# chlhnu/DOT-SOCP

Hardware: AMD Instinct MI355X
Metric: ADMM iters/sec on NxNxT dot2d staggered grid at 1/2/4/8 MI355X (higher is better)
Workload: dtype f64

## Files before the change

dot-socp_amd/capi.py:

```python
import ctypes
import os

import numpy as np

_HERE = os.path.dirname(os.path.abspath(__file__))
LIB_PATH = os.path.join(_HERE, "lib", "libdotsocp.so")

i64 = ctypes.c_longlong
dbl = ctypes.c_double
vp = ctypes.c_void_p


class DotsocpError(RuntimeError):
    def __init__(self, code, msg):
        super().__init__(f"libdotsocp error {code}: {msg}")
        self.code = code


class Problem(ctypes.Structure):
    _fields_ = [("dim", ctypes.c_int), ("weighted", ctypes.c_int),
                ("ny", i64), ("nx", i64), ("nt", i64),
                ("D", dbl), ("E", dbl), ("cScale", dbl), ("dScale", dbl),
                ("normc", dbl), ("normd", dbl)]

# ... 82 lines not shown
    "dotsocp_bfd_conj_dev": (ctypes.c_int, [vp, vp, i64, i64, i64, dbl, vp]),
    "dotsocp_create": (vp, [ctypes.POINTER(Problem), ctypes.c_int, ctypes.c_int]),
    "dotsocp_create_multi": (vp, [ctypes.POINTER(Problem), ctypes.c_int, ctypes.c_int]),
    "dotsocp_destroy": (None, [vp]),
    "dotsocp_rccl_unique_id": (ctypes.c_int, [vp]),
    "dotsocp_attach_rccl": (ctypes.c_int, [vp, vp, ctypes.c_int, ctypes.c_int]),
    "dotsocp_slab_range": (ctypes.c_int, [i64, ctypes.c_int, ctypes.c_int, ctypes.POINTER(i64), ctypes.POINTER(i64)]),
    "dotsocp_field_len": (i64, [ctypes.POINTER(Problem), ctypes.c_int]),
    "dotsocp_dct_algorithm": (ctypes.c_int, [i64]),
    "dotsocp_dct_levels": (ctypes.c_int, [i64, ctypes.c_int]),
    "dotsocp_cdft_levels": (ctypes.c_int, [i64]),
    "dotsocp_tsolve_tri_safe": (ctypes.c_int, [i64, i64, i64]),
    "dotsocp_cone_writes_beta": (ctypes.c_int, [i64, dbl, i64, ctypes.c_int, ctypes.c_int, ctypes.c_int, dbl, dbl]),
    "dotsocp_rescale_due": (ctypes.c_int, [i64, ctypes.c_int, dbl, dbl]),
    "dotsocp_qcone_form": (ctypes.c_int, [i64, dbl, i64, ctypes.c_int, ctypes.c_int, ctypes.c_int, ctypes.c_int, dbl, dbl]),
    "dotsocp_release_cache": (i64, []),
    "dotsocp_upload": (ctypes.c_int, [vp, ctypes.c_int, vp]),
    "dotsocp_upload_layers": (ctypes.c_int, [vp, ctypes.c_int, vp, i64, i64]),
    "dotsocp_download": (ctypes.c_int, [vp, ctypes.c_int, vp]),
    "dotsocp_begin": (ctypes.c_int, [vp, ctypes.POINTER(Opts)]),
    "dotsocp_begin_method": (ctypes.c_int, [vp, ctypes.POINTER(Opts), ctypes.c_int, ctypes.POINTER(AccOpts)]),
    "dotsocp_run": (ctypes.c_int, [vp, i64, ctypes.POINTER(i64)]),
    "dotsocp_recover_outputs": (ctypes.c_int, [vp, vp, vp, vp, vp, vp, vp, vp, vp]),
    "dotsocp_report_edges": (ctypes.c_int, [vp]),
    "dotsocp_solution_report": (ctypes.c_int, [vp, vp, vp, ctypes.POINTER(Report), vp, vp]),
    "dotsocp_recover_velocity": (ctypes.c_int, [vp, vp, vp, dbl, vp, vp]),
    "dotsocp_advect_particles": (ctypes.c_int, [vp, vp, vp, ctypes.POINTER(AdvectOpts), vp, vp, vp, vp, ctypes.POINTER(i64)]),
    "dotsocp_push_mass": (ctypes.c_int, [vp, vp, vp, ctypes.POINTER(PushOpts), vp, vp, vp, vp, vp, ctypes.POINTER(i64),
                                         ctypes.POINTER(dbl), vp]),
    "dotsocp_map_report": (ctypes.c_int, [vp, vp, vp, ctypes.POINTER(AdvectOpts), vp, vp, vp, ctypes.POINTER(MapReport),
# ... 107 lines not shown
```

dot-socp_amd/csrc/capi.hip:

```cpp
#include <cstring>
#include <new>

#include "comm.h"
#include "image_table.h"
#include "solver.h"
#include "weights.h"

using namespace dotsocp;

namespace dotsocp {
extern thread_local std::string g_last_error;
int dotsocp_slab_range_impl(i64 nt, int world, int rank, i64 *t0, i64 *t1);
}

struct dotsocp_ctx {
    Solver s;
};

struct dotsocp_weights {
    Weights w;
};

static int require_device() {
    int n = 0;
// ... 263 lines not shown
int dotsocp_cdft_levels(dotsocp_i64 n) { return cdft_levels(n); }
int dotsocp_tsolve_tri_safe(dotsocp_i64 ny, dotsocp_i64 nx, dotsocp_i64 nt) { return tsolve_tri_safe(ny, nx, nt) ? 1 : 0; }

int dotsocp_cone_writes_beta(dotsocp_i64 it, double last_sigma_it, dotsocp_i64 maxit, int check_step_by_step,
                             int last_of_run, int rescale, double maxFeas, double relGap) {
    return cone_writes_beta(it, last_sigma_it, maxit, check_step_by_step != 0, last_of_run != 0, rescale, maxFeas, relGap) ? 1 : 0;
}
int dotsocp_rescale_due(dotsocp_i64 it, int rescale, double maxFeas, double relGap) {
    return rescale_due(it, rescale, maxFeas, relGap) ? 1 : 0;
}
int dotsocp_qcone_form(dotsocp_i64 it, double last_sigma_it, dotsocp_i64 maxit, int check_step_by_step, int last_of_run,
                       int next_last_of_run, int rescale, double maxFeas, double relGap) {
    return qcone_form(it, last_sigma_it, maxit, check_step_by_step != 0, last_of_run != 0, next_last_of_run != 0, rescale,
                      maxFeas, relGap);
}

dotsocp_i64 dotsocp_field_len(const dotsocp_problem *p, int field) {
    if (!p || (p->dim != 1 && p->dim != 2) || p->nt < 2 || p->nx < 1 || (p->dim == 2 && p->ny < 1)) return -1;
    const i64 ny = p->dim == 1 ? p->nx : p->ny, nx = p->dim == 1 ? 1 : p->nx, nt = p->nt;
    const i64 Nphi = ny * nx * nt, Nz = ny * nx * (nt - 1);
    const i64 Nq = Nz + ny * (nx - 1) * nt + (ny - 1) * nx * nt;
    switch (field) {
        case DOTSOCP_F_PHI: case DOTSOCP_F_C: return Nphi;
        case DOTSOCP_F_Q: case DOTSOCP_F_ALPHA: case DOTSOCP_F_WEIGHT: return Nq;
        case DOTSOCP_F_Z: case DOTSOCP_F_BETA: return Nz * (p->dim == 1 ? 6 : 10);
        default: return -1;
    }
}

int dotsocp_upload(dotsocp_ctx *ctx, int field, const double *host) { CTX_OR_FAIL(); return ctx->s.upload(field, host); }
// ... 223 lines not shown
```

dot-socp_amd/csrc/fused.hip:

```cpp
#include "device_utils.h"
#include "gather_tile.h"
#include "kernels.h"

#include <cstdlib>

namespace dotsocp {

template <int MODE, int XB, bool NT = false, bool GIN = false, bool GOUT = false>
__global__ void __launch_bounds__(64 * XB) k_cone_fused(Grid g, LoopCoef c, FusedArgs a) {
    static_assert(MODE == 1 || !(GIN || GOUT), "the gamma form exists between two MODE_B passes only");
    constexpr bool DUAL = (MODE >= 5);
    constexpr bool UPD = (MODE != 0 && MODE != 6);
    constexpr bool PROJ = (MODE < 2 || MODE >= 5);
    __shared__ double2 xch[2][XB][64];
    __shared__ double2 xchp[DUAL ? 2 : 1][DUAL ? XB : 1][DUAL ? 64 : 1];
    const int lane = threadIdx.x, xl = threadIdx.y;
    const BlockId blk = block_id(a.xcd != 0);
    const i64 y = (i64)blk.x * 64 + lane;
    const i64 x = (i64)blk.y * XB + xl;
    const bool inb = (y < g.ny) && (x < g.nx);
    const i64 yc = inb ? y : 0, xc = inb ? x : 0;
    const i64 t0 = ((i64)blk.z + a.z0) * a.TC;
    const i64 t1 = (t0 + a.TC < g.ncl) ? t0 + a.TC : g.ncl;
    const bool lastChunk = (t1 == g.ncl);
    constexpr bool GATHER = (PROJ || MODE == 4);
    const bool carried = GATHER && !DUAL && t0 > 0 && a.carry_in != nullptr;
    const i64 tstart = (GATHER && t0 > 0 && !carried) ? t0 - 1 : t0;
    const i64 nxblk = gridDim.y, nyblk = gridDim.x;

    EdgeQuad cur = load_edges(g, a.q, yc, xc, tstart, c.sf), curo, cur3;
    if (UPD && !GIN) curo = load_edges(g, a.q_old, yc, xc, tstart, c.sf);
    if (MODE == 5) cur3 = load_edges(g, a.q3, yc, xc, tstart, c.sf);
    GatherCarry gc, gcp;
    if (carried) {
        const i64 ci = yc + g.py * xc;
        gc.p3 = a.carry_in[ci]; gc.p4 = a.carry_in[g.plane + ci];
        gc.p7 = a.carry_in[2 * g.plane + ci]; gc.p8 = a.carry_in[3 * g.plane + ci];
    }
// ... 111 lines not shown
    fg.nxblk = (g.nx + fg.XB - 1) / fg.XB;
    const i64 tiles = fg.nyblk * fg.nxblk;
    const i64 target = 2048;
    i64 chunks = (target + tiles - 1) / tiles;
    if (chunks < 1) chunks = 1;
    if (!(g.first && g.last) && cone_split_enabled() && chunks < 2 && g.ncl >= 12) chunks = 2;
    i64 TC = (g.ncl + chunks - 1) / chunks;
    if (TC < 8) TC = 8;
    if (TC > g.ncl) TC = g.ncl;
    if (TC < 1) TC = 1;
    fg.TC = TC;
    fg.chunks = (g.ncl + TC - 1) / TC;
    fg.sx_len = (g.ncl + 1) * fg.nxblk * g.ny;
    fg.sy_len = (g.ncl + 1) * g.nx * fg.nyblk;
    return 0;
}

int launch_cone_fused(int mode, const Grid &g, const LoopCoef &c, const FusedGeom &fg, FusedArgs a,
                      hipStream_t st, i64 z0, i64 zcount, int flavour) {
    if (g.Nz <= 0) return 0;
    if (zcount < 0) zcount = fg.chunks - z0;
    if (z0 < 0 || zcount <= 0 || z0 + zcount > fg.chunks) return 0;
    a.TC = fg.TC;
    a.z0 = (int)z0;
    a.xcd = tile_xcd_remap(g) ? 1 : 0;
    dim3 grid((unsigned)fg.nyblk, (unsigned)fg.nxblk, (unsigned)zcount);
    dim3 blk(64, 4);
    const bool nt = stream_nt_enabled();
#define CONE_MODE(M)                                                                     \
    case M:                                                                              \
// ... 27 lines not shown
```

dot-socp_amd/csrc/kernels.h:

```cpp
#pragma once
#include "common.h"
#include "defer.h"
#include "particle_block.h"

namespace dotsocp {

struct LoopCoef {
    double s;
    double sf;
    double dF;
    double at, ax, ay;
    double tau;
    double c1, c2;
    double dinv1, dinv2;
};

enum {
    S_Q2 = 0, S_Z2, S_APHI2, S_ALPHA2, S_BETA2, S_FBBETA2, S_PRIM1, S_PRIM2, S_DUAL1, S_DUAL2,
    S_COMPLEM, S_DOTCOMP, S_RHO2, S_RHOFQ2, S_MRHOB, S_M2, S_RHOB2, S_QALPHA, S_CPHI, S_PHI2,
    S_COUNT
};

struct KktCoef {
    double sigma;
// ... 37 lines not shown
    const double *q_old;
    const double *q;
    const double *beta_in;
    double *beta_out;
    double *z_out;
    double *q2;
    double *sx, *sy;
    const double *q3;
    double *p2, *sxp, *syp;
    i64 TC;
    ScaleOps bops;
    int xcd;
    int z0;
    const double *carry_in;
    double *carry_out;
};
bool tile_xcd_remap(const Grid &g);
int fused_geometry(const Grid &g, FusedGeom &fg);
enum { CONE_GIN = 1, CONE_GOUT = 2 };
int launch_cone_fused(int mode, const Grid &g, const LoopCoef &c, const FusedGeom &fg, FusedArgs a,
                      hipStream_t st, i64 z0 = 0, i64 zcount = -1, int flavour = 0);
bool cone_split_enabled();

struct KktWork;
struct AccArgs {
    const double *q;
    const double *z_in, *beta_in;
    const double *z0, *beta0;
    double *z0_out, *beta0_out;
    double bdiv;
    KktCoef kk;
// ... 103 lines not shown
    int c_ends;
};
int launch_qstep_rhs(const Grid &g, const LoopCoef &c, const FusedGeom &fg, const double *phi, const double *q2,
                     const double *sx, const double *sy, const double *weight, const double *tail_bx,
                     const double *tail_by, const double *cvec, double *q_out, const double *alpha_in, double *alpha_out,
                     double *rhs, hipStream_t st, i64 z0 = 0, i64 zcount = -1, i64 zstride = 1,
                     const QStepExtra *ex = nullptr);
i64 qstep_rhs_blocks(const Grid &g, const FusedGeom &fg);
struct QConeArgs {
    const double *phi, *q2v, *sx, *sy, *cvec, *alpha_in, *gamma_in;
    double *alpha_out, *rhs, *q_out, *beta_out, *q2_out, *sx_out, *sy_out;
    i64 TC;
    int ap_on;
    double ap_mul, ap_div;
    int c_ends;
};
int launch_qcone(const Grid &g, const LoopCoef &c, const FusedGeom &fg, QConeArgs a, bool gout, hipStream_t st);
i64 qcone_chunk_len(const Grid &g);
i64 qstep_rhs_chunks(const Grid &g, const FusedGeom &fg, i64 *TC = nullptr);
int launch_qstep_rhs_acc(int var, const Grid &g, const LoopCoef &c, const FusedGeom &fg, const double *phi,
                         const double *q2, const double *sx, const double *sy, const double *weight, const double *cvec,
                         double *q_raw, const double *alpha_in, double *alpha_out, double *rhs, double *q_state,
                         const double *q_anchor, const double *alpha_anchor, const AccCoef &k, hipStream_t st,
                         const double *tail_bx = nullptr, const double *tail_by = nullptr, double *u0_tail = nullptr);
int launch_qstep_palm_first(const Grid &g, const LoopCoef &c, const FusedGeom &fg, const double *phi, const double *q2,
                            const double *sx, const double *sy, const double *cvec, double *q_out, const double *alpha,
                            double *rhs, hipStream_t st, const double *tail_bx = nullptr, const double *tail_by = nullptr,
                            const double *qk = nullptr);

int launch_qstep_fused(const Grid &g, const LoopCoef &c, const FusedGeom &fg, const double *phi,
                       const double *q2, const double *sx, const double *sy, const double *weight,
                       const double *tail_bx, const double *tail_by, double *q_out, double *alpha,
// ... 98 lines not shown
```

dot-socp_amd/csrc/qstep_march.hip:

```cpp
#include "device_utils.h"
#include "gather_tile.h"
#include "kernels.h"
#include "qstep_tile.h"

#include <cstdlib>

namespace dotsocp {


struct QRhsArgs {
    const double *phi, *q2v, *sx, *sy, *weight, *tail_bx, *tail_by, *cvec, *alpha_in;
    double *q_out, *alpha_out, *rhs;
    double *u0_tail;
    i64 TC, z0, zstride;
    double *q_state;
    const double *q_anchor, *alpha_anchor;
    double c1, c2, om_rho, rho;
    APend ap;
    int xcd;
    const double *qk;
    double *partials, *resid;
    double kappa, dsD;
    int c_ends;
};
// ... 252 lines not shown
#define QRHS_LAUNCH(W, V) DS_KLAUNCH((k_qstep_rhs<W, V>), grid, blk, 0, st, g, c, fg, a)
    if (var == 0 && a.partials) {
        if (a.weight) DS_KLAUNCH((k_qstep_rhs<true, 0, true>), grid, blk, 0, st, g, c, fg, a);
        else DS_KLAUNCH((k_qstep_rhs<false, 0, true>), grid, blk, 0, st, g, c, fg, a);
    } else if (a.weight) {
        if (var == 0) QRHS_LAUNCH(true, 0); else if (var == 1) QRHS_LAUNCH(true, 1); else QRHS_LAUNCH(true, 2);
    } else {
        if (var == 0) QRHS_LAUNCH(false, 0); else if (var == 1) QRHS_LAUNCH(false, 1);
        else if (var == 2) QRHS_LAUNCH(false, 2); else QRHS_LAUNCH(false, 3);
    }
#undef QRHS_LAUNCH
    DS_HIP(hipGetLastError());
    return 0;
}

template <bool NT, bool GOUT>
__global__ void __launch_bounds__(TILE_Y *TILE_X, 3) k_qcone(Grid g, LoopCoef c, FusedGeom fg, QConeArgs a) {
    constexpr int XB = TILE_X;
    __shared__ double2 xch[2][XB][TILE_Y];
    __shared__ double ph[2][XB + 2][TILE_Y + 2];
    __shared__ double2 gch[2][XB][64];
    const APend ap{a.ap_on, a.ap_mul, a.ap_div};
    const BlockId blk = block_id(true);
    const QTile<XB> t = q_tile<XB>(g, fg, blk);
    const int lane = t.lane, xl = t.xl;
    const i64 y = t.y, x = t.x;
    const bool inb = t.inb;
    const i64 t0 = (i64)blk.z * a.TC;
    const i64 t1 = (t0 + a.TC < g.ntl) ? t0 + a.TC : g.ntl;
    const i64 tstart = (t0 >= 2) ? t0 - 2 : 0;
    const i64 tstop = (t1 == g.ntl) ? t1 + 1 : t1;
    const i64 nxblk = gridDim.y, nyblk = gridDim.x;
    const QSrc src{a.phi, a.q2v, a.sx, a.sy, nullptr, nullptr, nullptr, a.cvec, a.alpha_in, nullptr, a.c_ends};
    double p0 = 0.0;
    if (inb) {
        const i64 node0 = y + g.py * (x + g.nx * tstart);
        p0 = a.phi[node0];
        store_phi_layer<XB>(ph[0], t, p0, load_phi_halo(g, t, a.phi, node0));
    }
    double u0prev = 0.0;
    double q0c = 0.0;
    EdgeQuad eprev{0.0, 0.0, 0.0, 0.0};
    GatherCarry gc;
    int par = 0;
    __syncthreads();
    for (i64 tl = tstart; tl < tstop; ++tl) {
        const bool own = tl >= t0;
        const bool hasC = (tl > tstart) && (tl - 1 < g.ncl);
        const i64 ci = t.yc + g.py * (t.xc + g.nx * (hasC ? tl - 1 : 0));
        double b[10];
        if (hasC) {
#pragma unroll
            for (int j = 0; j < 10; ++j) b[j] = ld_stream<NT>(a.gamma_in + j * g.Nc + ci);
        }
        EdgeQuad ecur{0.0, 0.0, 0.0, 0.0};
        double q0n = 0.0;
        if (tl < g.ntl) {
            const QLayerIn in = q_layer_load<false, XB>(g, c, fg, t, src, ph[par], tl, false, false);
            const QLayerOut o = q_layer_calc<false, 0, XB>(c, t, in, ap, p0, false, false);
            q0n = o.q0n;
            if (own) {
                if (in.hasCell) {
                    a.alpha_out[in.node] = o.a0n;
                    if (!GOUT) a.q_out[in.node] = o.q0n;
                }
                if (t.hasBx) {
                    a.alpha_out[in.eX] = o.aXn;
                    if (!GOUT) a.q_out[in.eX] = o.qXn;
                }
                if (t.hasBy) {
                    a.alpha_out[in.eY] = o.aYn;
                    if (!GOUT) a.q_out[in.eY] = o.qYn;
                }
            }
            xch[par][xl][lane] = make_double2(o.ubx, o.qXn);
            store_phi_layer<XB>(ph[par ^ 1], t, in.pTl, in.h);
            __syncthreads();
            const double uby_s = __shfl_up(o.uby, 1, 64);
            const double qY_s = __shfl_up(o.qYn, 1, 64);
            if (inb) {
                const double2 r = from_left(t, xch[par], make_double2(o.ubx_l, o.qL),
                                            make_double2(0.0, 0.0));
                const double uby_m = from_below(t, uby_s, o.uby_b), qY_m = from_below(t, qY_s, o.qB);
                if (own) a.rhs[in.node] = adjoint_sum(g, c, t, tl, u0prev, o.u0, r.x, o.ubx, uby_m, o.uby) + in.cv;
                ecur.xm = (x >= 1) ? c.sf * r.y : 0.0;
                ecur.xp = (x <= g.nx - 2) ? c.sf * o.qXn : 0.0;
                ecur.ym = (y >= 1) ? c.sf * qY_m : 0.0;
                ecur.yp = (y <= g.ny - 2) ? c.sf * o.qYn : 0.0;
            }
            u0prev = o.u0;
            p0 = o.pT;
            par ^= 1;
        }
        if (tl > tstart) {
            double w[10];
            if (hasC) {
                double v[10];
                build_z2(v, q0c, eprev, ecur, c.s, c.dF);
#pragma unroll
                for (int j = 0; j < 10; ++j) b[j] = mult_finish(b[j], v[j], c.tau);
                if (!GOUT && own && inb) {
#pragma unroll
                    for (int j = 0; j < 10; ++j) st_stream<NT>(a.beta_out + j * g.Nc + ci, b[j]);
                }
#pragma unroll
                for (int j = 0; j < 10; ++j) v[j] = v[j] - b[j];
                proj_row<10>(v);
                if (GOUT && own && inb) {
// ... 1 lines not shown
                    for (int j = 0; j < 10; ++j) st_stream<NT>(a.beta_out + j * g.Nc + ci, mult_carry(b[j], v[j], c.tau));
                }
#pragma unroll
                for (int j = 0; j < 10; ++j) w[j] = v[j] + b[j];
                if (own && inb) a.q2_out[ci] = c.s * (w[9] - w[0]);
            } else {
#pragma unroll
                for (int j = 0; j < 10; ++j) w[j] = 0.0;
            }
            gather_emit<XB>(g, c.sf, gch, gc, w, tl - 1, own && inb, x, y, xl, lane, nxblk, nyblk, blk.y, blk.x, a.q2_out,
                            a.sx_out, a.sy_out);
        }
        eprev = ecur;
        q0c = q0n;
    }
}

i64 qcone_chunk_len(const Grid &g) {
    i64 TC = g.ntl;
    if (const char *e = getenv("DOTSOCP_QCONE_TC")) {
        const i64 n = atoll(e);
        if (n >= 1) TC = n;
    }
    return TC < g.ntl ? TC : g.ntl;
}

int launch_qcone(const Grid &g, const LoopCoef &c, const FusedGeom &fg, QConeArgs a, bool gout, hipStream_t st) {
    if (fg.XB != TILE_X || !(g.first && g.last) || g.ncl < 1) { set_error("internal: k_qcone on a grid it does not serve"); return DOTSOCP_ESTATE; }
    a.TC = qcone_chunk_len(g);
    const i64 chunks = (g.ntl + a.TC - 1) / a.TC;
    dim3 grid((unsigned)fg.nyblk, (unsigned)fg.nxblk, (unsigned)chunks);
    dim3 blk(TILE_Y, TILE_X);
    const bool nt = stream_nt_enabled();
    if (gout) {
        if (nt) DS_KLAUNCH((k_qcone<true, true>), grid, blk, 0, st, g, c, fg, a);
        else DS_KLAUNCH((k_qcone<false, true>), grid, blk, 0, st, g, c, fg, a);
    } else {
        if (nt) DS_KLAUNCH((k_qcone<true, false>), grid, blk, 0, st, g, c, fg, a);
        else DS_KLAUNCH((k_qcone<false, false>), grid, blk, 0, st, g, c, fg, a);
    }
    DS_HIP(hipGetLastError());
    return 0;
}

int launch_qstep_palm_first(const Grid &g, const LoopCoef &c, const FusedGeom &fg, const double *phi, const double *q2,
                            const double *sx, const double *sy, const double *cvec, double *q_out, const double *alpha,
                            double *rhs, hipStream_t st, const double *tail_bx, const double *tail_by, const double *qk) {
    QRhsArgs a{};
// ... 7 lines not shown
```

dot-socp_amd/csrc/solver.h:

```cpp
#pragma once
#include <chrono>
#include <functional>
#include <memory>
#include <string>
#include <type_traits>
#include <vector>

#include "hostmem.h"
#include "kernels.h"

namespace dotsocp {

constexpr unsigned long long POISON_WORD = 0x7ff8bad0bad0bad0ull;
int guarded_malloc(void **p, size_t bytes, bool fp = false);
void guarded_free(void *p);
bool poison_enabled();
int poison_region(void *p, size_t bytes);
long long device_cache_release();
long long device_cache_held(int dev);
int canary_check(std::string *report);
bool canary_enabled();
bool stream_stress_enabled();
void stream_stress(hipStream_t st);

// ... 221 lines not shown
    bool deferred = false;
    bool z_valid = true;
    bool z_prev_ok = false;
    bool rhs_valid = false;
    bool cone_carry = true;
    bool beta_gamma = false;
    bool cone_gout = false;
    bool last_of_run = false;
    int qcone = -1;
    bool q_valid = true;
    bool early_pass = false;
    bool early_gout = false;
    bool next_last_of_run = false;
    int need_q(const char *who) const;
    int qcone_decide() const;
    bool time_limit_passed() const;
    i64 timeout_at = -1;
    bool timeout_pending = false;
    int need_beta_form(const char *who) const;
    ScaleOps bops{0, 1.0, 1.0, 1.0, 1.0};
    ScaleOps zp_ops{0, 1.0, 1.0, 1.0, 1.0};
    int push_beta_op(double mul, double div);
    int flush_beta();
    ScaleOps aops{0, 1.0, 1.0, 1.0, 1.0};
    int flush_alpha();
    int sigma_scale_folded(double factor);
    FusedArgs pending_step_args(const Slab &s) const;
    double last_S[S_COUNT] = {0};
    double last_S_sigma = 1.0;
    i64 last_S_it = -1;
// ... 73 lines not shown
```

dot-socp_amd/csrc/solver.hip:

```cpp
#include "solver.h"

#include <algorithm>
#include <cmath>
#include <cstring>

#include "comm.h"

namespace dotsocp {

void Solver::update_coef() {
    lc.s = E / D;
    lc.sf = edge_factor(lc.s);
    lc.dF = E / dScale;
    const double ht = 1.0 / (double)(nt - 1);
    lc.at = D * (1.0 / ht);
    lc.ax = (nx > 1) ? D * (1.0 / (1.0 / (double)(nx - 1))) : 0.0;
    lc.ay = (ny > 1) ? D * (1.0 / (1.0 / (double)(ny - 1))) : 0.0;
    lc.tau = opts.tau;
    const double tmp = (E / D) * (E / D);
    if (prob.weighted) { lc.c1 = 2.0 * tmp; lc.c2 = tmp; }
    else { lc.c1 = 1.0 + 2.0 * tmp; lc.c2 = 1.0 + tmp; }
    lc.dinv1 = 1.0 / lc.c1;
    lc.dinv2 = 1.0 / lc.c2;
}
// ... 246 lines not shown
        DS_CHECK(flush_alpha());
        FOR_SLABS(s) DS_CHECK(launch_rhs(s.g, lc, s.q, s.alpha, s.c, s.weight, s.u0_prev, s.w0, s.st, c_ends_on && s.c_ends));
    } else if (multi()) {
        FOR_SLABS(s)
            if (!s.g.first) DS_CHECK(launch_rhs_fixup(s.g, lc, s.u0_prev, s.w0, s.st));
    }
    rhs_valid = false;
    prof_end(PH_RHS);
    prof_begin(PH_POISSON);
    DS_CHECK(poisson_all(hooks));
    prof_end(PH_POISSON);
    return 0;
}

int Solver::phase_z(int part) {
    if (early_pass) {
        early_pass = false;
        if (part != 0 || !fused || !deferred || cone_gout != early_gout) {
            set_error("internal: the early cone pass wrote %s, the schedule asks for %s", early_gout ? "gamma" : "beta",
                      cone_gout ? "gamma" : "beta");
            return DOTSOCP_ESTATE;
        }
        return 0;
    }
    DS_CHECK(need_q("phase_z"));
    if (part != 1) DS_CHECK(ensure_halo());
    if (!fused) {
        prof_begin(PH_PROJ);
        FOR_SLABS(s) DS_CHECK(launch_cone_proj(s.g, lc, s.q, s.beta, s.z, s.st));
        prof_end(PH_PROJ);
        return 0;
    }
    const bool gin = beta_gamma, gout = deferred && cone_gout;
    if (gin && (!deferred || !bops.empty())) {
        set_error("internal: gamma form %s", deferred ? "with a pending scaling of beta" : "without a pending multiplier step");
        return DOTSOCP_ESTATE;
    }
    const int flavour = (gin ? CONE_GIN : 0) | (gout ? CONE_GOUT : 0);
    const int ph = deferred ? (gin ? PH_CONE_CARRY : PH_FUSED_B) : PH_FUSED_A;
    z_valid = false;
// ... 3 lines not shown
        FusedArgs a{};
        a.q = s.q;
        a.q2 = s.q2;
        a.sx = s.sx;
        a.sy = s.sy;
        a.beta_in = s.beta;
        a.bops = bops;
        const i64 C = s.fg.chunks;
        const i64 z0 = (part == 2) ? C - 1 : 0;
        const i64 zc = (part == 0) ? C : ((part == 1) ? C - 1 : 1);
        if (deferred) {
            a.q_old = s.q_old;
            a.beta_out = s.beta2;
        }
        const int mode = deferred ? 1 : 0;
        if (s.carry && C > 1) {
            for (i64 z = z0; z < z0 + zc; ++z) {
                a.carry_in = (z > 0) ? s.carry : nullptr;
                a.carry_out = (z + 1 < C) ? s.carry : nullptr;
                DS_CHECK(launch_cone_fused(mode, s.g, lc, s.fg, a, s.st, z, 1, flavour));
            }
        } else {
            DS_CHECK(launch_cone_fused(mode, s.g, lc, s.fg, a, s.st, z0, zc, flavour));
        }
        if (deferred && part != 1) std::swap(s.beta, s.beta2);
    }
    prof_end(ph);
    if (part == 1) return 0;
    if (deferred) {
        bops.clear();
        beta_gamma = gout;
    }
    return 0;
}

KktCoef Solver::kkt_coef() const {
    KktCoef k;
    k.sigma = sigma;
    k.kappa = sigma * cScale * D;
    k.dsD = dScale / D;
    k.dsE = dScale / E;
    return k;
}

int Solver::phase_q(int part, bool kkt, int early) {
    if (!fused) DS_CHECK(flush_alpha());
    if (early != QCONE_NONE && (part != 0 || kkt || multi() || !fused || !deferred || !beta_gamma || !bops.empty())) {
        set_error("internal: early cone pass in a state it does not serve");
        return DOTSOCP_ESTATE;
    }
    const bool egout = (early == QCONE_STEADY);
    const int ph = (early != QCONE_NONE) ? PH_QCONE : PH_QSTEP;
    prof_begin(ph);
    FOR_SLABS(s) {
        hipStream_t st = s.st;
        if (early != QCONE_NONE && qcone != 2) {
            if (!s.sx2) {
                DS_CHECK(s.zalloc(&s.sx2, s.fg.sx_len));
                DS_CHECK(s.zalloc(&s.sy2, s.fg.sy_len));
            }
            QConeArgs a{};
            a.phi = s.phi; a.q2v = s.q2; a.sx = s.sx; a.sy = s.sy; a.cvec = s.c; a.alpha_in = s.alpha; a.gamma_in = s.beta;
            a.alpha_out = s.alpha2; a.rhs = s.w0; a.q_out = s.q_old; a.beta_out = s.beta2;
            a.q2_out = s.q; a.sx_out = s.sx2; a.sy_out = s.sy2;
            a.ap_on = aops.n; a.ap_mul = aops.mul; a.ap_div = aops.div;
            a.c_ends = (c_ends_on && s.c_ends) ? 1 : 0;
            DS_CHECK(launch_qcone(s.g, lc, s.fg, a, egout, st));
            std::swap(s.alpha, s.alpha2);
            std::swap(s.q, s.q_old);
            std::swap(s.q2, s.q_old);
            std::swap(s.sx, s.sx2);
// ... 8 lines not shown
            else if (part == 2) { z0 = C - 1; zc = 1; }
            QStepExtra ex{};
            ex.aops = aops;
            ex.c_ends = (c_ends_on && s.c_ends) ? 1 : 0;
            if (multi() && !s.g.last && part != 1) ex.u0_tail = s.send_plane;
            if (kkt) {
                const KktCoef k = kkt_coef();
                ex.partials = kkt_qstep_partials(s.g, s.kw);
                ex.resid = s.w1;
                ex.kappa = k.kappa; ex.dsD = k.dsD;
            }
            DS_CHECK(launch_qstep_rhs(s.g, lc, s.fg, s.phi, s.q2, s.sx, s.sy, s.weight, s.tail_bx, s.tail_by, s.c,
                                      s.q_old, s.alpha, s.alpha2, s.w0, st, z0, zc, zs, &ex));
            if (part != 1) std::swap(s.alpha, s.alpha2);
            if (part != 1) std::swap(s.q, s.q_old);
            if (early != QCONE_NONE) {
                FusedArgs a{};
                a.q = s.q; a.q2 = s.q2; a.sx = s.sx; a.sy = s.sy;
                a.beta_in = s.beta; a.beta_out = s.beta2;
                a.bops = bops;
                DS_CHECK(launch_cone_fused(1, s.g, lc, s.fg, a, s.st, 0, s.fg.chunks, CONE_GIN | (egout ? CONE_GOUT : 0)));
                std::swap(s.beta, s.beta2);
            }
        }
    }
    prof_end(ph);
    if (part == 1) return 0;
    q_valid = true;
    if (early != QCONE_NONE) {
        q_valid = !egout || qcone == 2;
        beta_gamma = egout;
        z_valid = false;
        z_prev_ok = false;
        early_pass = true;
        early_gout = egout;
    }
    u0_made = multi() && fused;
    if (fused) aops.clear();
    rhs_valid = fused;
    if (multi() && fused && comm_z && cone_split_enabled()) halo_pending = true;
    else DS_CHECK(exchange_q_halo(true));
    return 0;
}

int Solver::phase_mult() {
    if (fused) {
// ... 216 lines not shown
    if (last_of_run) return true;
    return rescale_due(it + 1, rescale, maxFeas, relGap);
}

int qcone_form(i64 it, double lastSigmaIt, i64 maxit, bool checkStepByStep, bool last_of_run, bool next_last_of_run,
               int rescale, double maxFeas, double relGap) {
    if (cone_writes_beta(it, lastSigmaIt, maxit, checkStepByStep, last_of_run, rescale, maxFeas, relGap)) return QCONE_NONE;
    return cone_writes_beta(it + 1, lastSigmaIt, maxit, checkStepByStep, next_last_of_run, rescale, maxFeas, relGap)
               ? QCONE_EXIT : QCONE_STEADY;
}

bool Solver::time_limit_passed() const {
    return timeout_pending || (remote() ? false : (elapsed() > time_limit || (timeout_at > 0 && it >= timeout_at)));
}

int Solver::qcone_decide() const {
    if (qcone == 0 || !fused || multi() || prob.weighted || method != DOTSOCP_METHOD_INPALM) return QCONE_NONE;
    if (!deferred || !beta_gamma || !bops.empty()) return QCONE_NONE;
    const Slab &s = slabs[0];
    if (s.g.ncl < 1 || s.fg.XB != 4) return QCONE_NONE;
    if (qcone < 0 && s.fg.nyblk * s.fg.nxblk < 2048) return QCONE_NONE;
    if (time_limit_passed()) return QCONE_NONE;
    return qcone_form(it, lastSigmaIt, opts.maxit, opts.ifCheckStepByStep != 0, last_of_run, next_last_of_run, rescale,
                      maxFeas, relGap);
}

bool if_adjust_sigma(double iter, double last_iter) {
    const double passed = iter - last_iter;
    if (iter < 20 && passed >= 3) return true;
    if (iter < 50 && passed >= 6) return true;
    if (iter < 100 && passed >= 10) return true;
    if (iter < 200 && passed >= 15) return true;
    if (iter < 500 && passed >= 25) return true;
    return passed >= 40;
}
// ... 130 lines not shown
            if (split) DS_CHECK(phase_z(2));
            return make_tails();
        };
        hooks.behind = [&]() -> int { return async_comm([&]() { return send_tails(); }, EV_JOIN); };
        DS_CHECK(phase_phi(&hooks));
    } else {
        DS_CHECK(phase_phi());
        DS_CHECK(phase_z(0));
    }
    if (fold) {
        FOR_SLABS(s) DS_CHECK(clear_partials(s));
    }
    if (inter) {
        DS_CHECK(async_comm([&]() { return send_phi_head(); }, EV_HALO));
        DS_CHECK(comm_wait(EV_JOIN));
        if (split_q) DS_CHECK(phase_q(1, fold));
        DS_CHECK(comm_wait(EV_HALO));
        DS_CHECK(phase_q(split_q ? 2 : 0, fold));
    } else {
        DS_CHECK(ship_tails());
        DS_CHECK(phase_q(0, fold, fold ? QCONE_NONE : qcone_decide()));
    }
    DS_CHECK(phase_mult());
    const bool timed_out = time_limit_passed();
    timeout_pending = false;
    if (timed_out && (beta_gamma || early_pass)) {
        timeout_pending = true;
        return 0;
    }
    if (kkt_due || timed_out)
        DS_CHECK(kkt_block(adjustSigmaYes, timed_out, brk, fold));
    return 0;
}
// ... 132 lines not shown
```

include/dotsocp.h:

```cpp
#ifndef DOTSOCP_H
#define DOTSOCP_H

#ifdef __cplusplus
extern "C" {
#endif

typedef long long dotsocp_i64;

enum {
    DOTSOCP_OK = 0,
    DOTSOCP_EINVAL = -1,
    DOTSOCP_ENODEVICE = -2,
    DOTSOCP_EHIP = -3,
    DOTSOCP_ESTATE = -4,
    DOTSOCP_ECOMM = -5
};

const char *dotsocp_last_error(void);
const char *dotsocp_version(void);
int dotsocp_device_count(void);
dotsocp_i64 dotsocp_release_cache(void);


int dotsocp_proj_soc(double *out, const double *in, dotsocp_i64 M, dotsocp_i64 K);
// ... 87 lines not shown
dotsocp_i64 dotsocp_field_len(const dotsocp_problem *prob, int field);

int dotsocp_dct_algorithm(dotsocp_i64 n);

int dotsocp_cdft_levels(dotsocp_i64 n);

int dotsocp_dct_levels(dotsocp_i64 n, int axis);

int dotsocp_tsolve_tri_safe(dotsocp_i64 ny, dotsocp_i64 nx, dotsocp_i64 nt);

int dotsocp_cone_writes_beta(dotsocp_i64 it, double last_sigma_it, dotsocp_i64 maxit, int check_step_by_step,
                             int last_of_run, int rescale, double maxFeas, double relGap);
int dotsocp_rescale_due(dotsocp_i64 it, int rescale, double maxFeas, double relGap);
int dotsocp_qcone_form(dotsocp_i64 it, double last_sigma_it, dotsocp_i64 maxit, int check_step_by_step, int last_of_run,
                       int next_last_of_run, int rescale, double maxFeas, double relGap);

int dotsocp_upload(dotsocp_ctx *ctx, int field, const double *host);
int dotsocp_download(dotsocp_ctx *ctx, int field, double *host);
int dotsocp_upload_layers(dotsocp_ctx *ctx, int field, const double *host, dotsocp_i64 t0, dotsocp_i64 n);

int dotsocp_begin(dotsocp_ctx *ctx, const dotsocp_opts *opts);
int dotsocp_begin_method(dotsocp_ctx *ctx, const dotsocp_opts *opts, int method, const dotsocp_acc_opts *acc);
int dotsocp_run(dotsocp_ctx *ctx, dotsocp_i64 n_iters, dotsocp_i64 *done);
int dotsocp_finish(dotsocp_ctx *ctx, dotsocp_result *res);

int dotsocp_recover_outputs(dotsocp_ctx *ctx, const double *rho0, const double *rho1, double *rho, double *Ex,
                            double *Ey, double *q0, double *bx, double *by);

#define DOTSOCP_REPORT_BINS 49
#define DOTSOCP_REPORT_RHO_FLOOR 1e-8
// ... 136 lines not shown
```

Measured before the change: 98.98.

## Extend fused q-step/cone early pass to multi-GPU slabs with split launches

Enables the fused qcone early pass, which combines the q-step and the cone projection, when the grid is split into slabs across multiple GPUs. The interior slab part runs the fused kernel before the halo arrives. The remaining tail layers are projected by a partial cone launch with t_begin/t_end bounds and a carry buffer. The aim is to remove a separate full cone pass and its memory traffic on multi-device runs, at the cost of more launch bookkeeping and schedule state.

```diff
diff --git a/dot-socp_amd/capi.py b/dot-socp_amd/capi.py
--- a/dot-socp_amd/capi.py
+++ b/dot-socp_amd/capi.py
@@ -120,6 +120,7 @@
     "dotsocp_cone_writes_beta": (ctypes.c_int, [i64, dbl, i64, ctypes.c_int, ctypes.c_int, ctypes.c_int, dbl, dbl]),
     "dotsocp_rescale_due": (ctypes.c_int, [i64, ctypes.c_int, dbl, dbl]),
     "dotsocp_qcone_form": (ctypes.c_int, [i64, dbl, i64, ctypes.c_int, ctypes.c_int, ctypes.c_int, ctypes.c_int, dbl, dbl]),
+    "dotsocp_cone_rest_launch": (ctypes.c_int, [i64, i64, i64, i64, ctypes.POINTER(i64), ctypes.POINTER(ctypes.c_int)]),
     "dotsocp_release_cache": (i64, []),
     "dotsocp_upload": (ctypes.c_int, [vp, ctypes.c_int, vp]),
     "dotsocp_upload_layers": (ctypes.c_int, [vp, ctypes.c_int, vp, i64, i64]),
diff --git a/dot-socp_amd/csrc/capi.hip b/dot-socp_amd/csrc/capi.hip
--- a/dot-socp_amd/csrc/capi.hip
+++ b/dot-socp_amd/csrc/capi.hip
@@ -301,6 +301,15 @@
     return qcone_form(it, last_sigma_it, maxit, check_step_by_step != 0, last_of_run != 0, next_last_of_run != 0, rescale,
                       maxFeas, relGap);
 }
+int dotsocp_cone_rest_launch(dotsocp_i64 ncl, dotsocp_i64 tc, dotsocp_i64 first, dotsocp_i64 z, dotsocp_i64 *t_begin,
+                             int *carried) {
+    i64 tb = 0;
+    int cr = 0;
+    const bool on = cone_rest_launch(ncl, tc, first, z, &tb, &cr);
+    if (t_begin) *t_begin = on ? tb : -1;
+    if (carried) *carried = on ? cr : 0;
+    return on ? 1 : 0;
+}
 
 dotsocp_i64 dotsocp_field_len(const dotsocp_problem *p, int field) {
     if (!p || (p->dim != 1 && p->dim != 2) || p->nt < 2 || p->nx < 1 || (p->dim == 2 && p->ny < 1)) return -1;
diff --git a/dot-socp_amd/csrc/fused.hip b/dot-socp_amd/csrc/fused.hip
--- a/dot-socp_amd/csrc/fused.hip
+++ b/dot-socp_amd/csrc/fused.hip
@@ -20,8 +20,10 @@
     const i64 x = (i64)blk.y * XB + xl;
     const bool inb = (y < g.ny) && (x < g.nx);
     const i64 yc = inb ? y : 0, xc = inb ? x : 0;
-    const i64 t0 = ((i64)blk.z + a.z0) * a.TC;
-    const i64 t1 = (t0 + a.TC < g.ncl) ? t0 + a.TC : g.ncl;
+    const i64 tc0 = ((i64)blk.z + a.z0) * a.TC;
+    const i64 t0 = (a.t_begin > tc0) ? a.t_begin : tc0;
+    const i64 tce = (a.t_end > 0 && a.t_end < g.ncl) ? a.t_end : g.ncl;
+    const i64 t1 = (tc0 + a.TC < tce) ? tc0 + a.TC : tce;
     const bool lastChunk = (t1 == g.ncl);
     constexpr bool GATHER = (PROJ || MODE == 4);
     const bool carried = GATHER && !DUAL && t0 > 0 && a.carry_in != nullptr;
@@ -163,6 +165,16 @@
     fg.sx_len = (g.ncl + 1) * fg.nxblk * g.ny;
     fg.sy_len = (g.ncl + 1) * g.nx * fg.nyblk;
     return 0;
+}
+
+bool cone_rest_launch(i64 ncl, i64 TC, i64 first, i64 z, i64 *t_begin, int *carried) {
+    if (TC < 1 || z < 0 || first < 0 || first >= ncl) return false;
+    const i64 c0 = z * TC, c1 = (c0 + TC < ncl) ? c0 + TC : ncl;
+    if (c0 >= ncl || c1 <= first) return false;
+    const i64 tb = (first > c0) ? first : c0;
+    if (t_begin) *t_begin = tb;
+    if (carried) *carried = (tb > 0) ? 1 : 0;
+    return true;
 }
 
 int launch_cone_fused(int mode, const Grid &g, const LoopCoef &c, const FusedGeom &fg, FusedArgs a,
diff --git a/dot-socp_amd/csrc/kernels.h b/dot-socp_amd/csrc/kernels.h
--- a/dot-socp_amd/csrc/kernels.h
+++ b/dot-socp_amd/csrc/kernels.h
@@ -75,7 +75,9 @@
     int z0;
     const double *carry_in;
     double *carry_out;
-};
+    i64 t_begin, t_end;
+};
+bool cone_rest_launch(i64 ncl, i64 TC, i64 first, i64 z, i64 *t_begin, int *carried);
 bool tile_xcd_remap(const Grid &g);
 int fused_geometry(const Grid &g, FusedGeom &fg);
 enum { CONE_GIN = 1, CONE_GOUT = 2 };
@@ -209,8 +211,12 @@
     int ap_on;
     double ap_mul, ap_div;
     int c_ends;
-};
-int launch_qcone(const Grid &g, const LoopCoef &c, const FusedGeom &fg, QConeArgs a, bool gout, hipStream_t st);
+    const double *tail_bx, *tail_by;
+    double *carry_out;
+    i64 t_lo, t_hi;
+};
+int launch_qcone(const Grid &g, const LoopCoef &c, const FusedGeom &fg, QConeArgs a, bool gout, hipStream_t st, i64 z0 = 0,
+                 i64 zcount = -1);
 i64 qcone_chunk_len(const Grid &g);
 i64 qstep_rhs_chunks(const Grid &g, const FusedGeom &fg, i64 *TC = nullptr);
 int launch_qstep_rhs_acc(int var, const Grid &g, const LoopCoef &c, const FusedGeom &fg, const double *phi,
diff --git a/dot-socp_amd/csrc/qstep_march.hip b/dot-socp_amd/csrc/qstep_march.hip
--- a/dot-socp_amd/csrc/qstep_march.hip
+++ b/dot-socp_amd/csrc/qstep_march.hip
@@ -290,7 +290,7 @@
     return 0;
 }
 
-template <bool NT, bool GOUT>
+template <bool NT, bool GOUT, bool SLAB = false>
 __global__ void __launch_bounds__(TILE_Y *TILE_X, 3) k_qcone(Grid g, LoopCoef c, FusedGeom fg, QConeArgs a) {
     constexpr int XB = TILE_X;
     __shared__ double2 xch[2][XB][TILE_Y];
@@ -302,12 +302,14 @@
     const int lane = t.lane, xl = t.xl;
     const i64 y = t.y, x = t.x;
     const bool inb = t.inb;
-    const i64 t0 = (i64)blk.z * a.TC;
-    const i64 t1 = (t0 + a.TC < g.ntl) ? t0 + a.TC : g.ntl;
+    const i64 thi = SLAB ? a.t_hi : g.ntl;
+    const i64 t0 = (SLAB ? a.t_lo : 0) + (i64)blk.z * a.TC;
+    const i64 t1 = (t0 + a.TC < thi) ? t0 + a.TC : thi;
     const i64 tstart = (t0 >= 2) ? t0 - 2 : 0;
     const i64 tstop = (t1 == g.ntl) ? t1 + 1 : t1;
     const i64 nxblk = gridDim.y, nyblk = gridDim.x;
-    const QSrc src{a.phi, a.q2v, a.sx, a.sy, nullptr, nullptr, nullptr, a.cvec, a.alpha_in, nullptr, a.c_ends};
+    const QSrc src{a.phi, a.q2v, a.sx, a.sy, nullptr, SLAB ? a.tail_bx : nullptr, SLAB ? a.tail_by : nullptr, a.cvec, a.alpha_in,
+                   nullptr, a.c_ends};
     double p0 = 0.0;
     if (inb) {
         const i64 node0 = y + g.py * (x + g.nx * tstart);
@@ -320,7 +322,50 @@
     GatherCarry gc;
     int par = 0;
     __syncthreads();
-    for (i64 tl = tstart; tl < tstop; ++tl) {
+    auto qpart = [&](const i64 tl, const bool own, const bool tails, EdgeQuad &ecur, double &q0n) {
+        const QLayerIn in = q_layer_load<false, XB>(g, c, fg, t, src, ph[par], tl, tails, false);
+        const QLayerOut o = q_layer_calc<false, 0, XB>(c, t, in, ap, p0, tails, false);
+        q0n = o.q0n;
+        const bool qst = !GOUT || (SLAB && (tl == 0 || tl == thi - 1));
+        if (own) {
+            if (in.hasCell) {
+                a.alpha_out[in.node] = o.a0n;
+                if (qst) a.q_out[in.node] = o.q0n;
+            }
+            if (t.hasBx) {
+                a.alpha_out[in.eX] = o.aXn;
+                if (qst) a.q_out[in.eX] = o.qXn;
+            }
+            if (t.hasBy) {
+                a.alpha_out[in.eY] = o.aYn;
+                if (qst) a.q_out[in.eY] = o.qYn;
+            }
+        }
+        xch[par][xl][lane] = make_double2(o.ubx, o.qXn);
+        store_phi_layer<XB>(ph[par ^ 1], t, in.pTl, in.h);
+        __syncthreads();
+        const double uby_s = __shfl_up(o.uby, 1, 64);
+        const double qY_s = __shfl_up(o.qYn, 1, 64);
+        if (inb) {
+            const double2 r = from_left(t, xch[par], make_double2(o.ubx_l, o.qL),
+                                        make_double2(0.0, 0.0));
+            const double uby_m = from_below(t, uby_s, o.uby_b), qY_m = from_below(t, qY_s, o.qB);
+            if (own) a.rhs[in.node] = adjoint_sum(g, c, t, tl, u0prev, o.u0, r.x, o.ubx, uby_m, o.uby) + in.cv;
+            ecur.xm = (x >= 1) ? c.sf * r.y : 0.0;
+            ecur.xp = (x <= g.nx - 2) ? c.sf * o.qXn : 0.0;
+            ecur.ym = (y >= 1) ? c.sf * qY_m : 0.0;
+            ecur.yp = (y <= g.ny - 2) ? c.sf * o.qYn : 0.0;
+        }
+        u0prev = o.u0;
+        p0 = o.pT;
+        par ^= 1;
+    };
+    i64 tl = tstart;
+    if constexpr (SLAB) {
+        qpart(tl, tl >= t0, (tl == 0) && !g.first, eprev, q0c);
+        ++tl;
+    }
+    for (; tl < tstop; ++tl) {
         const bool own = tl >= t0;
         const bool hasC = (tl > tstart) && (tl - 1 < g.ncl);
         const i64 ci = t.yc + g.py * (t.xc + g.nx * (hasC ? tl - 1 : 0));
@@ -331,43 +376,7 @@
         }
         EdgeQuad ecur{0.0, 0.0, 0.0, 0.0};
         double q0n = 0.0;
-        if (tl < g.ntl) {
-            const QLayerIn in = q_layer_load<false, XB>(g, c, fg, t, src, ph[par], tl, false, false);
-            const QLayerOut o = q_layer_calc<false, 0, XB>(c, t, in, ap, p0, false, false);
-            q0n = o.q0n;
-            if (own) {
-                if (in.hasCell) {
-                    a.alpha_out[in.node] = o.a0n;
-                    if (!GOUT) a.q_out[in.node] = o.q0n;
-                }
-                if (t.hasBx) {
-                    a.alpha_out[in.eX] = o.aXn;
-                    if (!GOUT) a.q_out[in.eX] = o.qXn;
-                }
-                if (t.hasBy) {
-                    a.alpha_out[in.eY] = o.aYn;
-                    if (!GOUT) a.q_out[in.eY] = o.qYn;
-                }
-            }
-            xch[par][xl][lane] = make_double2(o.ubx, o.qXn);
-            store_phi_layer<XB>(ph[par ^ 1], t, in.pTl, in.h);
-            __syncthreads();
-            const double uby_s = __shfl_up(o.uby, 1, 64);
-            const double qY_s = __shfl_up(o.qYn, 1, 64);
-            if (inb) {
-                const double2 r = from_left(t, xch[par], make_double2(o.ubx_l, o.qL),
-                                            make_double2(0.0, 0.0));
-                const double uby_m = from_below(t, uby_s, o.uby_b), qY_m = from_below(t, qY_s, o.qB);
-                if (own) a.rhs[in.node] = adjoint_sum(g, c, t, tl, u0prev, o.u0, r.x, o.ubx, uby_m, o.uby) + in.cv;
-                ecur.xm = (x >= 1) ? c.sf * r.y : 0.0;
-                ecur.xp = (x <= g.nx - 2) ? c.sf * o.qXn : 0.0;
-                ecur.ym = (y >= 1) ? c.sf * qY_m : 0.0;
-                ecur.yp = (y <= g.ny - 2) ? c.sf * o.qYn : 0.0;
-            }
-            u0prev = o.u0;
-            p0 = o.pT;
-            par ^= 1;
-        }
+        if (tl < g.ntl) qpart(tl, own, false, ecur, q0n);
         if (tl > tstart) {
             double w[10];
             if (hasC) {
@@ -399,6 +408,11 @@
         eprev = ecur;
         q0c = q0n;
     }
+    if (SLAB && t1 == thi && inb) {
+        const i64 ci = y + g.py * x;
+        a.carry_out[ci] = gc.p3; a.carry_out[g.plane + ci] = gc.p4;
+        a.carry_out[2 * g.plane + ci] = gc.p7; a.carry_out[3 * g.plane + ci] = gc.p8;
+    }
 }
 
 i64 qcone_chunk_len(const Grid &g) {
@@ -410,13 +424,40 @@
     return TC < g.ntl ? TC : g.ntl;
 }
 
-int launch_qcone(const Grid &g, const LoopCoef &c, const FusedGeom &fg, QConeArgs a, bool gout, hipStream_t st) {
-    if (fg.XB != TILE_X || !(g.first && g.last) || g.ncl < 1) { set_error("internal: k_qcone on a grid it does not serve"); return DOTSOCP_ESTATE; }
+int launch_qcone(const Grid &g, const LoopCoef &c, const FusedGeom &fg, QConeArgs a, bool gout, hipStream_t st, i64 z0,
+                 i64 zcount) {
+    const bool slab = !(g.first && g.last);
+    bool ok = (fg.XB == TILE_X) && g.ncl >= 1;
+    a.t_lo = 0;
+    a.t_hi = g.ntl;
+    if (slab) {
+        i64 TCq = 1;
+        const i64 Cq = qstep_rhs_chunks(g, fg, &TCq);
+        ok = ok && z0 >= 0 && zcount >= 1 && z0 + zcount < Cq && (g.first || (a.tail_bx && a.tail_by)) && a.carry_out;
+        a.t_lo = z0 * TCq;
+        a.t_hi = (z0 + zcount) * TCq;
+        ok = ok && a.t_hi < g.ntl && a.t_hi - 1 < g.ncl && a.t_hi - a.t_lo >= 2;
+    } else {
+        ok = ok && z0 == 0 && zcount < 0;
+    }
+    if (!ok) { set_error("internal: k_qcone on a grid it does not serve"); return DOTSOCP_ESTATE; }
     a.TC = qcone_chunk_len(g);
-    const i64 chunks = (g.ntl + a.TC - 1) / a.TC;
+    if (a.TC > a.t_hi - a.t_lo) a.TC = a.t_hi - a.t_lo;
+    const i64 chunks = (a.t_hi - a.t_lo + a.TC - 1) / a.TC;
     dim3 grid((unsigned)fg.nyblk, (unsigned)fg.nxblk, (unsigned)chunks);
     dim3 blk(TILE_Y, TILE_X);
     const bool nt = stream_nt_enabled();
+    if (slab) {
+        if (gout) {
+            if (nt) DS_KLAUNCH((k_qcone<true, true, true>), grid, blk, 0, st, g, c, fg, a);
+            else DS_KLAUNCH((k_qcone<false, true, true>), grid, blk, 0, st, g, c, fg, a);
+        } else {
+            if (nt) DS_KLAUNCH((k_qcone<true, false, true>), grid, blk, 0, st, g, c, fg, a);
+            else DS_KLAUNCH((k_qcone<false, false, true>), grid, blk, 0, st, g, c, fg, a);
+        }
+        DS_HIP(hipGetLastError());
+        return 0;
+    }
     if (gout) {
         if (nt) DS_KLAUNCH((k_qcone<true, true>), grid, blk, 0, st, g, c, fg, a);
         else DS_KLAUNCH((k_qcone<false, true>), grid, blk, 0, st, g, c, fg, a);
diff --git a/dot-socp_amd/csrc/solver.h b/dot-socp_amd/csrc/solver.h
--- a/dot-socp_amd/csrc/solver.h
+++ b/dot-socp_amd/csrc/solver.h
@@ -259,6 +259,8 @@
     bool next_last_of_run = false;
     int need_q(const char *who) const;
     int qcone_decide() const;
+    i64 qcone_slab_first(const Slab &s) const;
+    bool qcone_slabs_ok() const;
     bool time_limit_passed() const;
     i64 timeout_at = -1;
     bool timeout_pending = false;
diff --git a/dot-socp_amd/csrc/solver.hip b/dot-socp_amd/csrc/solver.hip
--- a/dot-socp_amd/csrc/solver.hip
+++ b/dot-socp_amd/csrc/solver.hip
@@ -284,16 +284,18 @@
 }
 
 int Solver::phase_z(int part) {
+    const bool rest = early_pass && multi();
     if (early_pass) {
-        early_pass = false;
-        if (part != 0 || !fused || !deferred || cone_gout != early_gout) {
+        if (!rest) early_pass = false;
+        if ((rest ? (part == 0 || !beta_gamma) : part != 0) || !fused || !deferred || cone_gout != early_gout) {
             set_error("internal: the early cone pass wrote %s, the schedule asks for %s", early_gout ? "gamma" : "beta",
                       cone_gout ? "gamma" : "beta");
             return DOTSOCP_ESTATE;
         }
-        return 0;
-    }
-    DS_CHECK(need_q("phase_z"));
+        if (!rest) return 0;
+    } else {
+        DS_CHECK(need_q("phase_z"));
+    }
     if (part != 1) DS_CHECK(ensure_halo());
     if (!fused) {
         prof_begin(PH_PROJ);
@@ -327,7 +329,16 @@
             a.beta_out = s.beta2;
         }
         const int mode = deferred ? 1 : 0;
-        if (s.carry && C > 1) {
+        if (rest) {
+            const i64 first = qcone_slab_first(s);
+            for (i64 z = z0; z < z0 + zc; ++z) {
+                int carried = 0;
+                if (!cone_rest_launch(s.g.ncl, s.fg.TC, first, z, &a.t_begin, &carried)) continue;
+                a.carry_in = carried ? s.carry : nullptr;
+                a.carry_out = (z + 1 < C) ? s.carry : nullptr;
+                DS_CHECK(launch_cone_fused(mode, s.g, lc, s.fg, a, s.st, z, 1, flavour));
+            }
+        } else if (s.carry && C > 1) {
             for (i64 z = z0; z < z0 + zc; ++z) {
                 a.carry_in = (z > 0) ? s.carry : nullptr;
                 a.carry_out = (z + 1 < C) ? s.carry : nullptr;
@@ -340,6 +351,7 @@
     }
     prof_end(ph);
     if (part == 1) return 0;
+    early_pass = false;
     if (deferred) {
         bops.clear();
         beta_gamma = gout;
@@ -358,16 +370,51 @@
 
 int Solver::phase_q(int part, bool kkt, int early) {
     if (!fused) DS_CHECK(flush_alpha());
-    if (early != QCONE_NONE && (part != 0 || kkt || multi() || !fused || !deferred || !beta_gamma || !bops.empty())) {
+    const bool eslab = (early != QCONE_NONE) && multi();
+    if (early != QCONE_NONE && ((eslab ? part == 0 : part != 0) || kkt || !fused || !deferred || !beta_gamma || !bops.empty())) {
         set_error("internal: early cone pass in a state it does not serve");
         return DOTSOCP_ESTATE;
     }
     const bool egout = (early == QCONE_STEADY);
-    const int ph = (early != QCONE_NONE) ? PH_QCONE : PH_QSTEP;
+    const int ph = (early != QCONE_NONE && part != 2) ? PH_QCONE : PH_QSTEP;
     prof_begin(ph);
     FOR_SLABS(s) {
         hipStream_t st = s.st;
-        if (early != QCONE_NONE && qcone != 2) {
+        if (eslab && part == 1) {
+            if (!s.sx2) {
+                DS_CHECK(s.zalloc(&s.sx2, s.fg.sx_len));
+                DS_CHECK(s.zalloc(&s.sy2, s.fg.sy_len));
+            }
+            const i64 Cq = qstep_rhs_chunks(s.g, s.fg);
+            if (qcone != 2) {
+                QConeArgs a{};
+                a.phi = s.phi; a.q2v = s.q2; a.sx = s.sx; a.sy = s.sy; a.cvec = s.c; a.alpha_in = s.alpha; a.gamma_in = s.beta;
+                a.alpha_out = s.alpha2; a.rhs = s.w0; a.q_out = s.q_old; a.beta_out = s.beta2;
+                a.q2_out = s.q; a.sx_out = s.sx2; a.sy_out = s.sy2;
+                a.ap_on = aops.n; a.ap_mul = aops.mul; a.ap_div = aops.div;
+                a.c_ends = (c_ends_on && s.c_ends) ? 1 : 0;
+                a.tail_bx = s.tail_bx;
+                a.tail_by = s.tail_by;
+                a.carry_out = s.carry;
+                DS_CHECK(launch_qcone(s.g, lc, s.fg, a, egout, st, 0, Cq - 1));
+            } else {
+                QStepExtra ex{};
+                ex.aops = aops;
+                ex.c_ends = (c_ends_on && s.c_ends) ? 1 : 0;
+                DS_CHECK(launch_qstep_rhs(s.g, lc, s.fg, s.phi, s.q2, s.sx, s.sy, s.weight, s.tail_bx, s.tail_by, s.c,
+                                          s.q_old, s.alpha, s.alpha2, s.w0, st, 0, Cq - 1, 1, &ex));
+                FusedArgs a{};
+                a.q = s.q_old; a.q2 = s.q; a.sx = s.sx2; a.sy = s.sy2;
+                a.beta_in = s.beta; a.beta_out = s.beta2;
+                a.bops = bops;
+                a.t_end = qcone_slab_first(s);
+                for (i64 z = 0; z * s.fg.TC < a.t_end; ++z) {
+                    a.carry_in = (z > 0) ? s.carry : nullptr;
+                    a.carry_out = s.carry;
+                    DS_CHECK(launch_cone_fused(1, s.g, lc, s.fg, a, st, z, 1, CONE_GIN | (egout ? CONE_GOUT : 0)));
+                }
+            }
+        } else if (early != QCONE_NONE && qcone != 2 && !eslab) {
             if (!s.sx2) {
                 DS_CHECK(s.zalloc(&s.sx2, s.fg.sx_len));
                 DS_CHECK(s.zalloc(&s.sy2, s.fg.sy_len));
@@ -406,7 +453,11 @@
                                       s.q_old, s.alpha, s.alpha2, s.w0, st, z0, zc, zs, &ex));
             if (part != 1) std::swap(s.alpha, s.alpha2);
             if (part != 1) std::swap(s.q, s.q_old);
-            if (early != QCONE_NONE) {
+            if (eslab) {
+                std::swap(s.q2, s.q_old);
+                std::swap(s.sx, s.sx2);
+                std::swap(s.sy, s.sy2);
+            } else if (early != QCONE_NONE) {
                 FusedArgs a{};
                 a.q = s.q; a.q2 = s.q2; a.sx = s.sx; a.sy = s.sy;
                 a.beta_in = s.beta; a.beta_out = s.beta2;
@@ -421,7 +472,7 @@
     q_valid = true;
     if (early != QCONE_NONE) {
         q_valid = !egout || qcone == 2;
-        beta_gamma = egout;
+        if (!eslab) beta_gamma = egout;
         z_valid = false;
         z_prev_ok = false;
         early_pass = true;
@@ -668,11 +719,29 @@
     return timeout_pending || (remote() ? false : (elapsed() > time_limit || (timeout_at > 0 && it >= timeout_at)));
 }
 
+i64 Solver::qcone_slab_first(const Slab &s) const {
+    i64 TCq = 1;
+    const i64 Cq = qstep_rhs_chunks(s.g, s.fg, &TCq);
+    return (Cq - 1) * TCq - 1;
+}
+
+bool Solver::qcone_slabs_ok() const {
+    if (!(comm_z && multi() && fused && cone_split_enabled())) return false;
+    for (const auto &s : slabs) {
+        if (s.g.ncl < 12 || s.fg.chunks < 2 || qstep_rhs_chunks(s.g, s.fg) < 2 || !s.carry) return false;
+        const i64 first = qcone_slab_first(s);
+        if (first < 1 || first >= s.g.ncl) return false;
+    }
+    return true;
+}
+
 int Solver::qcone_decide() const {
-    if (qcone == 0 || !fused || multi() || prob.weighted || method != DOTSOCP_METHOD_INPALM) return QCONE_NONE;
+    if (qcone == 0 || !fused || prob.weighted || method != DOTSOCP_METHOD_INPALM) return QCONE_NONE;
+    if (multi() && !qcone_slabs_ok()) return QCONE_NONE;
     if (!deferred || !beta_gamma || !bops.empty()) return QCONE_NONE;
     const Slab &s = slabs[0];
-    if (s.g.ncl < 1 || s.fg.XB != 4) return QCONE_NONE;
+    for (const auto &o : slabs)
+        if (o.g.ncl < 1 || o.fg.XB != 4) return QCONE_NONE;
     if (qcone < 0 && s.fg.nyblk * s.fg.nxblk < 2048) return QCONE_NONE;
     if (time_limit_passed()) return QCONE_NONE;
     return qcone_form(it, lastSigmaIt, opts.maxit, opts.ifCheckStepByStep != 0, last_of_run, next_last_of_run, rescale,
@@ -833,9 +902,10 @@
     if (inter) {
         DS_CHECK(async_comm([&]() { return send_phi_head(); }, EV_HALO));
         DS_CHECK(comm_wait(EV_JOIN));
-        if (split_q) DS_CHECK(phase_q(1, fold));
+        const int early = (split && split_q && !fold) ? qcone_decide() : QCONE_NONE;
+        if (split_q) DS_CHECK(phase_q(1, fold, early));
         DS_CHECK(comm_wait(EV_HALO));
-        DS_CHECK(phase_q(split_q ? 2 : 0, fold));
+        DS_CHECK(phase_q(split_q ? 2 : 0, fold, early));
     } else {
         DS_CHECK(ship_tails());
         DS_CHECK(phase_q(0, fold, fold ? QCONE_NONE : qcone_decide()));
diff --git a/include/dotsocp.h b/include/dotsocp.h
--- a/include/dotsocp.h
+++ b/include/dotsocp.h
@@ -125,6 +125,8 @@
 int dotsocp_rescale_due(dotsocp_i64 it, int rescale, double maxFeas, double relGap);
 int dotsocp_qcone_form(dotsocp_i64 it, double last_sigma_it, dotsocp_i64 maxit, int check_step_by_step, int last_of_run,
                        int next_last_of_run, int rescale, double maxFeas, double relGap);
+int dotsocp_cone_rest_launch(dotsocp_i64 ncl, dotsocp_i64 tc, dotsocp_i64 first, dotsocp_i64 z, dotsocp_i64 *t_begin,
+                             int *carried);
 
 int dotsocp_upload(dotsocp_ctx *ctx, int field, const double *host);
 int dotsocp_download(dotsocp_ctx *ctx, int field, double *host);
```

Result: slower. 97.97 (-1.0%).
